# kmkolasinski/tfrecords-reader

Hardware: AMD Instinct MI355X
Metric: GiB/s + examples/s device-resident TFRecord->Feature decode, 1/2/4/8 GPU (higher is better)
Workload: dtype u8; 1 GPU; C4 directory (configs[4]) of 256 files, C1-shaped (int64 label + 12 B bytes_list id) records, 524288 +-50 % per file (default_rng(1000+f)), spec CRC-32C; this rank's LPT share (256 files) resident in HBM; records_per_gpu=134295581, framed_bytes_per_gpu=7906235019, parallelism=file-sharded x1 (LPT by bytes, no collective on the data path), batches_per_gpu=4, batch_bytes_max=1976558779, streams=2, tpl_groups_missed=0

## Files before the change

tfrecords-reader_amd/csrc/tfrg_capi.cpp:

```cpp
#include <hip/hip_runtime.h>
#include <stdlib.h>
#include <string.h>

#include <algorithm>
#include <map>
#include <numeric>
#include <string>
#include <unordered_map>
#include <vector>

#include "../../include/tfrg.h"
#include "crc32c.h"
#include "tfrg_internal.h"

namespace tfrg {
void set_error(const std::string& s);

#define HIP_TRY(expr)                                                              \
  do {                                                                             \
    hipError_t e_ = (expr);                                                        \
    if (e_ != hipSuccess) {                                                        \
      set_error(std::string(#expr) + ": " + hipGetErrorString(e_));               \
      return TFRG_E_HIP;                                                           \
    }                                                                              \
// ... 48 lines not shown
  const uint32_t* s32 = nullptr;
  const uint32_t* e32 = nullptr;
  uint32_t first = 0;
  uint32_t mode = kOffU64;
};

struct tfrg_ctx {
  int device = 0;
  hipStream_t own_stream = nullptr;
  hipStream_t last_stream = nullptr;
  uint32_t lane_max = 2048;
  uint32_t wave_stage = 0xffffffffu;
  uint64_t record_bound = 0;
  uint64_t call_bound = 0;
  int num_cus = 256;
  DBuf crc_tab, consts;
  DBuf ht, key_hash, key_off, key_blob, key_slot, slot_kind, key_w, krec;
  uint32_t n_keys = 0, n_slots = 0, ht_mask = 0;
  DBuf in_bytes, in_start, in_end;
  DBuf status, aux, verdict, order, count, loc, rs, slot_base, totals, kind_totals;
  DBuf ident;
  size_t ident_n = 0;
  DBuf i64, f32, b_off, b_len, big_list, slow_list, miss, info, tsum, crc_rec, crc_base, crc_part;
  DBuf dq, dq_cnt;
  DBuf lmask, rlist;
  DBuf bdata, boff64, blb, bbig;
  bool materialized = false;
  bool tsum_dirty = true;
  uint32_t info_slot = 0;
  bool info_clean = false;
  uint32_t n = 0;
  uint64_t cap_hint = 0;
  hipEvent_t order_ev = nullptr;
  uint64_t nbytes = 0;
  uint64_t cap_i64 = 0, cap_f32 = 0, cap_b = 0;
  bool have_result = false;
  bool rs_complete = false;
  std::unordered_map<std::string, uint32_t> key_id;
  std::vector<int32_t> key_slot_h;
  DBuf tpl;
  uint32_t n_tpl = 0;
  uint32_t tpl_w = 0;
  size_t tpl_img_off = 0;
  uint32_t tpl_img_words = 0;
  std::vector<uint32_t> tpl_h;
  bool tpl_learned = false;
  bool tpl_full = false;
  bool tpl_on = true;
  std::vector<uint8_t> slot_kind_h;
  DBuf spec;
  std::vector<uint32_t> spec_h;
  bool have_spec = false;
  bool spec_on = true;
  bool profiling = false;
  bool have_events = false;
  hipEvent_t ev[kNumStages + 1] = {};
  uint64_t hint_i64 = 0, hint_f32 = 0, hint_b = 0;
  bool hinted = false;
  bool no_hints = false;
// ... 25 lines not shown
extern "C" {

int tfrg_ctx_create(int device, tfrg_ctx** out) {
  *out = nullptr;
  int ndev = 0;
  HIP_TRY(hipGetDeviceCount(&ndev));
  if (device < 0 || device >= ndev) {
    set_error("bad device index");
    return TFRG_E_ARG;
  }
  HIP_TRY(hipSetDevice(device));
  tfrg_ctx* c = new tfrg_ctx();
  c->device = device;
  if (const char* e = getenv("TFRG_TEMPLATES")) c->tpl_on = atoi(e) != 0;
  if (const char* e = getenv("TFRG_SPEC")) c->spec_on = atoi(e) != 0;
  if (const char* e = getenv("TFRG_OPTIMISTIC")) c->optimistic_on = atoi(e) != 0;
  if (const char* e = getenv("TFRG_WALK_BESIDE")) c->walk_beside = atoi(e) != 0;
  if (const char* e = getenv("TFRG_WALK_BLOCKS")) c->walk_blocks = (uint32_t)atoi(e);
  if (const char* e = getenv("TFRG_DEBUG_POISON_LOC")) {
    char* q = const_cast<char*>(e);
    for (int i = 0; i < 4 && *q; ++i) {
      c->poison[i] = (uint32_t)strtoul(q, &q, 10);
      while (*q == ',' || *q == ' ') ++q;
    }
  }
  hipDeviceProp_t prop;
  if (hipGetDeviceProperties(&prop, device) == hipSuccess) c->num_cus = prop.multiProcessorCount;
  if (hipStreamCreateWithFlags(&c->own_stream, hipStreamNonBlocking) != hipSuccess) {
    delete c;
    set_error("hipStreamCreate failed");
    return TFRG_E_HIP;
  }
  if (hipHostMalloc(reinterpret_cast<void**>(&c->info_pin), (kInfoCount + 8) * 4) != hipSuccess) {
    (void)hipStreamDestroy(c->own_stream);
    delete c;
    set_error("hipHostMalloc failed");
    return TFRG_E_NOMEM;
  }
  std::vector<uint32_t> tab(kLeanTabOff + 32 * 256), cst(128);
  CrcTables T;
  crc_make_tables(&T);
  memcpy(tab.data(), T.t, 4096);
  uint32_t M[4][256];
  crc_make_mul_tables(gf_xpow8(1024), M);
  memcpy(tab.data() + 1024, M, 4096);
  memcpy(tab.data() + 2048, T.t, 8192);
  memcpy(tab.data() + 4096, T.t, 16384);
  for (int e = 0; e < 256; ++e)
    for (int col = 0; col < 47; ++col) tab[8192 + e * 64 + col] = T.t[(col + 1) & 15][e];
  crc_make_mul_tables(gf_xpow8(2048), M);
  memcpy(tab.data() + 24576, M, 4096);
  crc_make_mul_tables(gf_xpow8(4096), M);
  memcpy(tab.data() + 25600, M, 4096);
  for (int k = 0; k < 24; ++k) {
    crc_make_mul_tables(gf_xpow8(1024ull << k), M);
    memcpy(tab.data() + 26624 + k * 1024, M, 4096);
  }
  for (int l = 0; l < 64; ++l) cst[l] = gf_xpow8(16ull * l);
  for (int z = 0; z < 16; ++z) cst[64 + z] = gf_xpow8_inv((uint64_t)z);
  for (int k = 0; k < 32; ++k) cst[96 + k] = gf_xpow8(1024ull << k);
  for (int v = 0; v < 256; ++v) {
    uint32_t x = T.t[0][v];
    for (int d = 0; d < 32; ++d) {
      tab[kLeanTabOff + d * 256 + v] = x;
      x = (x >> 8) ^ T.t[0][x & 0xff];
    }
  }
  if (c->crc_tab.ensure(tab.size() * 4) != hipSuccess || c->consts.ensure(cst.size() * 4) != hipSuccess ||
      hipMemcpy(c->crc_tab.p, tab.data(), tab.size() * 4, hipMemcpyHostToDevice) != hipSuccess ||
      hipMemcpy(c->consts.p, cst.data(), cst.size() * 4, hipMemcpyHostToDevice) != hipSuccess) {
    set_error("constant upload failed");
    tfrg_ctx_destroy(c);
    return TFRG_E_HIP;
  }
  *out = c;
  return 0;
}

int tfrg_ctx_destroy(tfrg_ctx* c) {
  if (!c) return 0;
  (void)hipSetDevice(c->device);
  if (c->last_stream) (void)hipStreamSynchronize(c->last_stream);
// ... 164 lines not shown
  DevSchema s;
  s.n_keys = c->n_keys;
  s.n_slots = c->n_slots;
  s.ht_mask = c->ht_mask;
  s.ht = c->ht.as<uint32_t>();
  s.key_hash = c->key_hash.as<uint32_t>();
  s.key_off = c->key_off.as<uint32_t>();
  s.key_blob = c->key_blob.as<uint8_t>();
  s.key_slot = c->key_slot.as<int32_t>();
  s.slot_kind = c->slot_kind.as<uint8_t>();
  s.key_w = c->key_w.as<uint32_t>();
  s.krec = c->krec.as<uint32_t>();
  s.tpl = c->tpl.as<uint32_t>();
  s.tpl_img = s.tpl + c->tpl_img_off;
  s.tpl_img_words = c->tpl_img_words;
  s.n_tpl = c->tpl_on ? c->n_tpl : 0u;
  s.tpl_w = c->tpl_w;
  s.spec = c->spec_on && c->have_spec ? c->spec.as<uint32_t>() : nullptr;
  return s;
}

namespace {

bool tpl_hdr2(const uint8_t* p, uint32_t L, uint32_t pos, uint32_t end, uint32_t& fn, uint32_t& off, uint32_t& len) {
  if (pos >= L || (p[pos] & 0x87u) != 0x02u) return false;
  fn = (p[pos] >> 3) & 0xfu;
  uint32_t q = pos + 1, l = 0;
  for (uint32_t nb = 0;; ++nb) {
    if (nb == 3 || q >= L) return false;
    const uint32_t b = p[q++];
// ... 93 lines not shown
        mode = 1;
      }
      if (mode) {
        cw = 1u | kCountInline;
        a = c0o;
        b = c0l;
      }
    }
    t.ent.insert(t.ent.end(), {(uint32_t)slot | (mode << 24), rank, cw, a | (b << 16)});
  }
  return !t.ent.empty();
}

struct Learned {
  std::vector<uint32_t> w, spec, img;
  uint32_t W = 0;
  bool have_spec = false;
  bool full = false;
  bool ord_const = false;
  bool len_const = false;
  std::vector<uint32_t> const_len;
};
uint32_t learn_shapes(const TplSchema* c, uint32_t S, const uint8_t* h_bytes, uint64_t nbytes, const uint64_t* h_start,
                      const uint64_t* h_end, uint32_t n, uint32_t flags, Learned& out) {
  std::map<std::string, std::pair<uint32_t, Tpl>> seen;
  Tpl t;
  const uint32_t lim = n < 4096u ? n : 4096u;
  for (uint32_t j = 0; j < lim; ++j) {
    const uint32_t i = (uint32_t)((uint64_t)j * n / lim);
    uint64_t a = h_start[i], e = h_end[i];
// ... 147 lines not shown
      }
      if (k == 0) sq |= kLiQSingle;
      if ((z[2] & ~kCountInline) > 1u) sq &= ~kLiQSingle;
    }
    img[3] |= d[kLtCrcw];
    img[4] = std::min(img[4], d[kLtChain]);
    if (lut[L] == 0xffu) {
      lut[L] = (uint8_t)k;
    } else {
      uint32_t p = lut[L];
      while (img[kLiTpl + (size_t)p * tw + 2] != 0xffu) p = img[kLiTpl + (size_t)p * tw + 2];
      img[kLiTpl + (size_t)p * tw + 2] = k;
    }
  }
  memcpy(&img[kLiLut], lut.data(), lut.size());
  out.ord_const = S > 0 && S <= kLeanMaxSlots;
  for (uint32_t s2 = 0; out.ord_const && s2 < S; ++s2) {
    const uint32_t r0 = w[kLtSlot + 3 * s2] >> 16;
    out.ord_const = r0 != 0;
    for (uint32_t k = 1; out.ord_const && k < nt; ++k) out.ord_const = (w[(size_t)k * kLtWords + kLtSlot + 3 * s2] >> 16) == r0;
  }
  out.len_const = S > 0 && S <= kLeanMaxSlots;
  out.const_len.assign(S, 0u);
  for (uint32_t s2 = 0; out.len_const && s2 < S; ++s2) {
    if ((c->slot_kind[s2] & 3u) != TFRG_KIND_BYTES) continue;
    const uint32_t z0 = w[kLtSlot + 3 * s2];
    out.len_const = (z0 & 0xffu) == 3u && (z0 >> 16) != 0;
    for (uint32_t k = 1; out.len_const && k < nt; ++k) {
      const uint32_t zk = w[(size_t)k * kLtWords + kLtSlot + 3 * s2];
      out.len_const = (zk & 0xffu) == 3u && (zk >> 16) != 0 && ((zk >> 8) & 0xffu) == ((z0 >> 8) & 0xffu);
    }
    out.const_len[s2] = (z0 >> 8) & 0xffu;
  }
  out.w = std::move(w);
  out.spec = std::move(spec);
  out.img = std::move(img);
  out.W = W;
  out.have_spec = have_spec;
  return nt;
}

bool learn_single_slots(const TplSchema* c, uint32_t S, const uint8_t* h_bytes, uint64_t nbytes,
                        const uint64_t* h_start, const uint64_t* h_end, uint32_t n, uint32_t flags,
                        std::vector<uint32_t>& spec) {
  spec.assign(S ? S : 1, 0u);
  if (!S || !n) return false;
  tfrg_host_ctx* hc = nullptr;
  if (tfrg_host_ctx_create(&hc)) return false;
  std::vector<uint32_t> single(S, 0u);
  uint32_t m = 0;
  const uint32_t lim = n < 4096u ? n : 4096u;
// ... 62 lines not shown
      set_error("template allocation failed");
      return TFRG_E_NOMEM;
    }
    HIP_TRY(hipMemcpy(c->spec.p, spec.data(), (size_t)c->n_slots * 4, hipMemcpyHostToDevice));
    c->spec_h = spec;
    c->have_spec = true;
    return 0;
  }
  const uint32_t S = c->n_slots;
  const std::vector<uint32_t>& w = L.w;
  const bool have_spec = L.have_spec;
  const std::vector<uint32_t>& spec = L.spec;
  const uint32_t W = L.W;
  HIP_TRY(hipSetDevice(c->device));
  if (c->last_stream) HIP_TRY(hipStreamSynchronize(c->last_stream));
  if (c->tpl.ensure((w.size() + L.img.size()) * 4) || (have_spec && c->spec.ensure((size_t)S * 4))) {
    set_error("template allocation failed");
    return TFRG_E_NOMEM;
  }
  HIP_TRY(hipMemcpy(c->tpl.p, w.data(), w.size() * 4, hipMemcpyHostToDevice));
  HIP_TRY(hipMemcpy(c->tpl.as<uint32_t>() + w.size(), L.img.data(), L.img.size() * 4, hipMemcpyHostToDevice));
  c->tpl_img_off = w.size();
  c->tpl_img_words = (uint32_t)L.img.size();
  if (have_spec) HIP_TRY(hipMemcpy(c->spec.p, spec.data(), (size_t)S * 4, hipMemcpyHostToDevice));
  c->n_tpl = nt;
  c->tpl_w = W;
  c->tpl_h = w;
  c->spec_h = spec;
  c->have_spec = have_spec;
  c->tpl_full = L.full;
  c->ord_const = L.ord_const;
  c->len_const = L.len_const;
  c->const_len = L.const_len;
  return (int)nt;
}

extern "C" int tfrg_learn_templates_host(uint32_t n_keys, const uint8_t* key_blob, const uint64_t* key_offsets,
                                         const uint32_t* key_flags, uint32_t n_slots, const uint32_t* slot_key,
// ... 204 lines not shown
  o.info = info_cur;
  o.info_next = c->info.as<uint32_t>() + (islot ^ 1u) * kInfoCount;
  o.tsum = c->tsum.as<uint32_t>();
  o.tile_stride = tile_stride;
  o.spine_lb = reinterpret_cast<uint64_t*>(o.tsum + (size_t)S * tile_stride);
  o.n_chunks = n_chunks;
  o.irr = o.tsum + (size_t)S * tile_stride + 2ull * S * n_chunks;
  o.slow_list = c->slow_list.as<uint32_t>();
  o.crc_rec = c->crc_rec.as<uint32_t>();
  o.crc_base = c->crc_base.as<uint64_t>();
  o.crc_part = c->crc_part.as<uint64_t>();
  o.lmask = c->lmask.as<uint64_t>();
  o.rlist = c->rlist.as<uint32_t>();
  LaunchCfg cfg;
  cfg.num_cus = c->num_cus;
  cfg.lean = c->tpl_on && c->n_tpl;
  cfg.tpl_full = cfg.lean && c->tpl_full;
  cfg.spec_h = c->spec_h.empty() ? nullptr : c->spec_h.data();
  const uint64_t lane_blocks = (n + 255) / 256;
  const uint64_t lane_cap = (uint64_t)c->num_cus * 8;
  cfg.lane_grid = (int)(lane_blocks < 1 ? 1 : (lane_blocks < lane_cap ? lane_blocks : lane_cap));
  const uint64_t wave_cap = (uint64_t)c->num_cus * 4;
  const uint64_t wave_blocks = (n + 3) / 4;
  cfg.wave_grid = (int)(wave_blocks < 1 ? 1 : (wave_blocks < wave_cap ? wave_blocks : wave_cap));
  cfg.lane_max = c->lane_max;
  cfg.wave_stage = c->wave_stage;
  memcpy(cfg.poison, c->poison, sizeof(cfg.poison));
  cfg.optimistic = c->optimistic_on && !c->no_quiet && c->poison[0] == 0xffffffffu;
  cfg.walk_beside = c->walk_beside;
  cfg.walk_blocks = c->walk_blocks;
// ... 311 lines not shown
```

tfrecords-reader_amd/csrc/tfrg_internal.h:

```cpp
#pragma once
#include <stdint.h>
#include <hip/hip_runtime.h>

namespace tfrg {

struct DevSchema {
  uint32_t n_keys;
  uint32_t n_slots;
  uint32_t ht_mask;
  const uint32_t* ht;
  const uint32_t* key_hash;
  const uint32_t* key_off;
  const uint8_t* key_blob;
  const int32_t* key_slot;
  const uint8_t* slot_kind;
  const uint32_t* key_w;
  const uint32_t* krec;
  const uint32_t* tpl;
  const uint32_t* tpl_img;
  uint32_t tpl_img_words;
  uint32_t n_tpl;
  uint32_t tpl_w;
  const uint32_t* spec;
};

constexpr uint32_t kTplMaxL = 240, kTplMaxEntries = 16;
constexpr uint32_t kLtMaxW = 64;
constexpr uint32_t kLeanMaxSlots = 16;
constexpr uint32_t kLtL = 0, kLtNe = 1, kLtCrcw = 2, kLtChain = 3, kLtK = 4, kLtAbsent = 5, kLtEnt = 8,
                   kLtWin = kLtEnt + 4 * kTplMaxEntries, kLtSlot = kLtWin + 3 * kLtMaxW,
                   kLtWords = kLtSlot + 3 * kLeanMaxSlots;
constexpr uint32_t kLeanTabOff = 51200;

constexpr uint32_t kTplMaxLane = 32;
constexpr uint32_t kLiHdr = 8, kLiSlotQ = kLiHdr, kLiLut = kLiSlotQ + kLeanMaxSlots,
                   kLiLutWords = (kTplMaxL + 1 + 3) / 4, kLiTpl = (kLiLut + kLiLutWords + 3) & ~3u;
constexpr uint32_t kLiQValue = 1u << 16, kLiQSingle = 1u << 17;
__host__ __device__ constexpr uint32_t kLiTw(uint32_t W) { return 4 + 3 * W + 4 * kLeanMaxSlots; }
constexpr uint32_t kLiMaxWords = (65536u - 32768u - 512u) / 4u;

struct LeanTgt {
  uint16_t* ord;
  uint32_t* cnt;
  uint2* loc;
  uint32_t* rs;
  void* v1;
  uint32_t* v2;
  uint32_t lim;
  uint32_t kind;
  uint32_t pad[2];
};
struct LeanArgs {
  uint32_t n_tpl;
  uint32_t lane_max;
  uint32_t* tsum;
  uint32_t n_slots;
  uint32_t tile_stride;
  uint32_t img_words;
  uint32_t gpw;
  uint32_t bsplit;
  uint32_t gsplit;
  const uint8_t* finish;
  uint32_t implicit;
  LeanTgt tg[kLeanMaxSlots];
};

enum KeyRec : uint32_t { kKrHash = 0, kKrLen, kKrW0, kKrW1, kKrSlot1, kKrSlot2, kKrSlot3, kKrFlags, kKrWords };
constexpr uint32_t kLdsMaxKeys = 256;
constexpr uint32_t kLdsMaxHt = 1024;

__host__ __device__ inline uint32_t key_hash_words(uint32_t n, uint32_t w0, uint32_t w1) {
  const uint32_t a = (w0 ^ (w0 >> 11) ^ (n << 17)) & 0xffffffu;
  const uint32_t b = (w1 ^ (w1 >> 13) ^ (n << 7)) & 0xffffffu;
#if defined(__HIP_DEVICE_COMPILE__)
  uint32_t p0, p1;
  asm("v_mul_u32_u24 %0, %1, %2" : "=v"(p0) : "v"(a), "v"(0x9E3779u));
  asm("v_mul_u32_u24 %0, %1, %2" : "=v"(p1) : "v"(b), "v"(0x85EBCBu));
  uint32_t h = p0 ^ p1;
// ... 140 lines not shown
  int num_cus;
  bool lean;
  bool tpl_full;
  const uint32_t* spec_h;
  int lane_grid;
  int wave_grid;
  uint32_t lane_max;
  uint32_t wave_stage;
  bool body_count;
  uint32_t poison[4];
  bool optimistic;
  bool ran_optimistic;
  bool ord_const;
  bool len_const;
  bool ran_quiet_big;
  bool walk_beside;
  uint32_t walk_blocks;
  uint32_t implicit;
};

enum Stage : int { kStageTplLane = 0, kStageLaneCount, kStageBodyCount, kStageTailCount, kStageSpine,
                   kStageDownGather, kStageTailGather, kStageMaterialize, kNumStages };
extern const char* const kStageNames[kNumStages];

hipError_t launch_tpl_lane(const DevBatch& b, const DevOut& o, const LeanArgs& a, const uint32_t* img, uint32_t w,
                           const uint32_t* d_tab, int num_cus, hipStream_t st);
hipError_t launch_fill_placed_rows(uint32_t* rs, const uint32_t* info, uint32_t n_slots, uint32_t n, hipStream_t st);
hipError_t launch_stream_read(const void* d, uint64_t nbytes, uint32_t* sink, hipStream_t st, int variant);
hipError_t launch_decode(const DevBatch& b, const DevSchema& sc, const DevOut& o, LaunchCfg& cfg,
                         const uint32_t* d_crc_tables, const uint32_t* d_wave_consts, hipStream_t stream,
                         hipEvent_t* ev);

}
```

tfrecords-reader_amd/csrc/tfrg_kernels.hip:

```cpp
#include <hip/hip_runtime.h>
#include <algorithm>
#include <type_traits>
#include "tfrg_internal.h"
#include "crc32c.h"
#include "tfrg_walk.h"
#include "../../include/tfrg_status.h"

namespace tfrg {

#ifdef TFRG_PHASE_PROF
__device__ unsigned long long g_phase[32];
#define PHASE_MARK(t) const uint64_t t = __builtin_readcyclecounter()
#define PHASE_ADD(i, a, b) \
  do {                     \
    if (lane == 0) atomicAdd(&g_phase[i], (unsigned long long)((b) - (a))); \
  } while (0)
#else
#define PHASE_MARK(t) (void)0
#define PHASE_ADD(i, a, b) (void)0
#endif

struct Src {
  const uint8_t* buf;
  uint64_t p0;
// ... 3114 lines not shown
  const bool tail_gord = slow_tail > kLaneLdsBudget;
  const size_t tail_lds = std::max<size_t>(tail_gord ? 2048ull * 4 : slow_tail, (kTailFinishWord + 4) * 4);
  const size_t walk_lds = 256ull * kLaneSlice * 4 + S * kTailBlock * 4 + r16(S * kTailBlock * 2) + keys_lds + spec_lds;
  const bool walk_beside = quiet_big && cfg.walk_beside && walk_lds <= tail_lds;
  cfg.implicit = 0;
  DevOut ox = o;
  if (!lean) {
    ox.lmask = nullptr;
    ox.rlist = nullptr;
  }
  mark(kStageTplLane);
  if (lean) {
    LeanArgs a{};
    a.n_tpl = sc.n_tpl;
    a.img_words = sc.tpl_img_words;
    a.lane_max = cfg.lane_max;
    a.tsum = cfg.ran_optimistic ? nullptr : o.tsum;
    a.finish = cfg.ran_optimistic ? sc.slot_kind : nullptr;
    cfg.implicit = cfg.ran_optimistic ? TFRG_IMPLICIT_STATUS | (cfg.ord_const ? TFRG_IMPLICIT_ORDER : 0u) |
                                            (cfg.len_const ? TFRG_IMPLICIT_BYTES_LEN : 0u)
                                      : 0u;
    a.implicit = cfg.implicit;
    a.n_slots = (uint32_t)S;
    a.tile_stride = o.tile_stride;
    const uint64_t n = b.n;
    for (uint32_t k = 0; k < S; ++k) {
      LeanTgt& t = a.tg[k];
      t.ord = o.order + k * n;
      t.cnt = o.count + k * n;
      t.loc = o.loc + k * n;
      t.rs = o.rs + k * (n + 1);
      const uint32_t sw = scx.spec && cfg.spec_h ? cfg.spec_h[k] : 0u;
      if (sw) {
        const uint32_t kind = sw & 3u;
        const uint64_t base = n * ((sw >> 2) - 1u);
        const uint64_t cap = kind == TFRG_KIND_INT64 ? o.cap_i64 : kind == TFRG_KIND_FLOAT ? o.cap_f32 : o.cap_b;
        t.lim = cap > base ? (uint32_t)std::min<uint64_t>(cap - base, n) : 0u;
        t.kind = kind;
        if (kind == TFRG_KIND_INT64) t.v1 = o.i64 + base;
        else if (kind == TFRG_KIND_FLOAT) t.v1 = o.f32 + base;
        else t.v1 = o.b_off + base;
        t.v2 = o.b_len + base;
      }
    }
    const hipError_t e = launch_tpl_lane(b, ox, a, sc.tpl_img, sc.tpl_w, d_tab, cfg.num_cus, st);
    if (e != hipSuccess) return e;
  }
  if (cfg.ran_optimistic && !quiet_big) {
    for (int i = kStageLaneCount; i <= kStageMaterialize; ++i) mark(i);
    return hipGetLastError();
  }
  mark(kStageLaneCount);
  auto resident_grid = [&](const void* fn, size_t lds, bool cap = true) {
    int per_cu = 0;
    if (hipOccupancyMaxActiveBlocksPerMultiprocessor(&per_cu, fn, kLaneCountBlock, lds) != hipSuccess || per_cu < 1)
      per_cu = 1;
    const int g = per_cu * cfg.num_cus;
    int need = (int)(((int64_t)cfg.lane_grid * 256 + kLaneCountBlock - 1) / kLaneCountBlock);
    if (quiet) need = std::min(need, 64);
    return g < need || !cap ? g : need;
// ... 164 lines not shown
```

tfrecords-reader_amd/csrc/tfrg_tpl.hip:

```cpp
#include <hip/hip_runtime.h>
#include "tfrg_internal.h"
#include "crc32c.h"
#include "../../include/tfrg_status.h"

namespace tfrg {

namespace {

constexpr int kTplBlock = 512;
constexpr uint32_t kTplTabs = 32;
static_assert(4u * kTplTabs * 256u + 4u * kLiMaxWords + 512u <= 65536u, "lane image + CRC tables exceed LDS");
constexpr uint32_t kHitVerdict = TFRG_V_LEN_MATCH | TFRG_V_LEN_CRC | TFRG_V_DATA_CRC;

typedef __attribute__((address_space(4))) const uint32_t cu32;

__device__ __forceinline__ uint32_t rfl(uint32_t x) { return __builtin_amdgcn_readfirstlane(x); }

template <int K>
__device__ __forceinline__ uint32_t bx4(uint32_t x) {
  uint32_t r;
  const uint32_t two = 2u;
  if constexpr (K == 0)
    asm("v_lshlrev_b32_sdwa %0, %1, %2 dst_sel:DWORD dst_unused:UNUSED_PAD src0_sel:DWORD src1_sel:BYTE_0"
        : "=v"(r) : "v"(two), "v"(x));
  else if constexpr (K == 1)
    asm("v_lshlrev_b32_sdwa %0, %1, %2 dst_sel:DWORD dst_unused:UNUSED_PAD src0_sel:DWORD src1_sel:BYTE_1"
        : "=v"(r) : "v"(two), "v"(x));
  else if constexpr (K == 2)
    asm("v_lshlrev_b32_sdwa %0, %1, %2 dst_sel:DWORD dst_unused:UNUSED_PAD src0_sel:DWORD src1_sel:BYTE_2"
        : "=v"(r) : "v"(two), "v"(x));
  else
    asm("v_lshlrev_b32_sdwa %0, %1, %2 dst_sel:DWORD dst_unused:UNUSED_PAD src0_sel:DWORD src1_sel:BYTE_3"
        : "=v"(r) : "v"(two), "v"(x));
  return r;
}

__device__ __forceinline__ uint32_t xor3(uint32_t a, uint32_t b, uint32_t c) {
  return __builtin_amdgcn_bitop3_b32(a, b, c, 0x96);
}

template <int D>
__device__ __forceinline__ uint32_t tl(const uint32_t* tab, uint32_t bx) {
  return *reinterpret_cast<const uint32_t*>(reinterpret_cast<const uint8_t*>(tab) + D * 1024 + bx);
}

template <int D>
__device__ __forceinline__ uint32_t lin_word(const uint32_t* tab, uint32_t x) {
  return xor3(tl<D + 3>(tab, bx4<0>(x)), tl<D + 2>(tab, bx4<1>(x)), tl<D + 1>(tab, bx4<2>(x))) ^ tl<D>(tab, bx4<3>(x));
}

__device__ __forceinline__ uint32_t vgroups(uint32_t w, uint32_t m) {
  w &= m;
  return (w & 0x7fu) | ((w >> 1) & 0x3f80u) | ((w >> 2) & 0x1fc000u) | ((w >> 3) & 0xfe00000u);
}
__device__ __forceinline__ uint32_t bytes_mask(uint32_t nb) { return nb >= 4u ? 0xffffffffu : (1u << (nb << 3)) - 1u; }

typedef uint32_t u32x4 __attribute__((ext_vector_type(4)));

struct LaneOff {
  uint32_t s, e;
};

__device__ __forceinline__ uint32_t wave_sum(uint32_t x) {
// ... 14 lines not shown
    uint64_t acc[4] = {0, 0, 0, 0};
    for (uint32_t k = 0; k < n_slots; ++k) {
      const uint32_t kd = slot_kind[k] & 3u;
      o.slot_base[k] = acc[kd];
      acc[kd] += n;
    }
    for (int k = 0; k < 4; ++k) o.kind_totals[k] = acc[k];
    if (acc[TFRG_KIND_INT64] > o.cap_i64 || acc[TFRG_KIND_FLOAT] > o.cap_f32 || acc[TFRG_KIND_BYTES] > o.cap_b)
      o.info[kInfoOverflow] = 1u;
    const uint64_t pm = n_slots >= 64u ? ~0ull : (1ull << n_slots) - 1ull;
    o.info[kInfoPlacedLo] = (uint32_t)pm;
    o.info[kInfoPlacedHi] = (uint32_t)(pm >> 32);
  }
}

template <int W, int OM>
__global__ __launch_bounds__(kTplBlock, W == 16 ? 6 : (W == 32 ? 4 : 2)) void k_tpl_lane(
    DevBatch B, DevOut o, LeanArgs A, const uint32_t* __restrict__ img, const uint32_t* __restrict__ tabs) {
  static_assert(W == 16 || W == 32 || W == 64, "window words");
  typedef uint32_t wvec __attribute__((ext_vector_type(W)));
  __shared__ __attribute__((aligned(16))) uint32_t tab[kTplTabs * 256];
  extern __shared__ __attribute__((aligned(16))) uint32_t limg[];
  constexpr uint32_t kWaves = kTplBlock / 64;
  constexpr uint32_t kTw = kLiTw(W);
  const uint32_t lane = threadIdx.x & 63u, wib = rfl(threadIdx.x >> 6);
  cu32* gimg = (cu32*)img;
  const uint32_t crcw_u = gimg[3], chain_u = gimg[4];
  const uint8_t* lut = reinterpret_cast<const uint8_t*>(limg + kLiLut);
  const __amdgpu_buffer_rsrc_t rsrc =
      __builtin_amdgcn_make_buffer_rsrc(const_cast<uint8_t*>(B.bytes), (short)0, (int)(uint32_t)B.nbytes, 0x00020000);
  const uint32_t nb = (uint32_t)B.nbytes;
  const uint32_t ngroups = (B.n + 63u) >> 6;
  static_assert(kTileShift == 8, "4 groups of 64 records per tile");
  const bool tail = blockIdx.x >= A.bsplit;
  const uint32_t gpw = tail ? 2u : A.gpw;
  const uint32_t gbeg0 = tail ? A.gsplit + ((blockIdx.x - A.bsplit) * kWaves + wib) * 2u : (blockIdx.x * kWaves + wib) * gpw;
  const uint32_t gbeg = gbeg0 < ngroups ? gbeg0 : ngroups;
  const uint32_t gend = gbeg + gpw < ngroups ? gbeg + gpw : ngroups;
  const bool whole = (gpw & 3u) == 0u;

  auto offsets = [&](uint32_t g) -> LaneOff {
    LaneOff f{1u, 0u};
// ... 20 lines not shown
  auto in_batch = [&](uint32_t g, uint32_t s, uint32_t e) {
    return (g << 6) + lane < B.n && s <= e && e <= nb && e >= 16u;
  };
  auto window = [&](wvec& wn, const LaneOff& f) {
    const uint32_t e = f.e;
    const bool full = e >= 4u * W && e <= nb;
    const uint32_t voff = full ? e - 4u * W : 0xffffff00u;
#pragma unroll
    for (int q = 0; q < W / 4; ++q) {
      const u32x4 v = __builtin_bit_cast(u32x4, __builtin_amdgcn_raw_buffer_load_b128(rsrc, voff + 16u * q, 0, 0));
      wn[4 * q] = v.x;
      wn[4 * q + 1] = v.y;
      wn[4 * q + 2] = v.z;
      wn[4 * q + 3] = v.w;
    }
  };
  auto head_fix = [&](wvec& wn, const LaneOff& f, uint32_t g) {
    if (g != 0u) return;
    const uint32_t e = f.e;
    const bool full = e >= 4u * W && e <= nb;
    const bool head = in_batch(g, start_of(f), e) && !full;
    if (__ballot(head)) {
#pragma unroll
      for (int i = 0; i < W; ++i) {
        uint32_t x = 0;
#pragma unroll
        for (int b = 0; b < 4; ++b) {
          const int64_t p = (int64_t)e - 4 * W + 4 * i + b;
          if (head && p >= 0) x |= (uint32_t)__builtin_amdgcn_raw_buffer_load_b8(rsrc, (uint32_t)p, 0, 0) << (8 * b);
        }
// ... 28 lines not shown
      const u32x4 meta = *reinterpret_cast<const u32x4*>(tp);
      uint32_t diff = 0;
#pragma unroll
      for (int q = 0; q < W / 4; ++q) {
        const u32x4 bm = *reinterpret_cast<const u32x4*>(tp + 4 + 4 * q);
        const u32x4 mm = *reinterpret_cast<const u32x4*>(tp + 4 + W + 4 * q);
        diff |= ((w[4 * q] ^ bm.x) & mm.x) | ((w[4 * q + 1] ^ bm.y) & mm.y) | ((w[4 * q + 2] ^ bm.z) & mm.z) |
                ((w[4 * q + 3] ^ bm.w) & mm.w);
        if (q & 1) __builtin_amdgcn_sched_barrier(0);
      }
      const uint32_t* cm = tp + 4 + 2 * W;
      uint32_t c = 0;
      if (chain_u < (uint32_t)(W - 9)) {
#pragma unroll
        for (int i = 0; i < W - 9; ++i)
          if ((uint32_t)i >= chain_u) c = lin_word<0>(tab, c ^ (w[i] & cm[i]));
      }
      uint32_t lin = 0;
#define TFRG_LIN(j)                                                                                       \
  if (crcw_u & (1u << (j))) lin ^= lin_word<28 - 4 * (j)>(tab, (w[W - 9 + (j)] & cm[W - 9 + (j)]) ^ ((j) == 0 ? c : 0u));
      TFRG_LIN(0) TFRG_LIN(1) TFRG_LIN(2) TFRG_LIN(3) TFRG_LIN(4) TFRG_LIN(5) TFRG_LIN(6) TFRG_LIN(7)
#undef TFRG_LIN
      const bool ok = act && diff == 0u && crc_mask(lin ^ meta.y) == w[W - 1];
      tsel = ok ? cand : tsel;
      cand = act && !ok ? meta.z : 0xffu;
    }
    const bool hit = tsel != 0xffu;
    if (hit && !(A.implicit & TFRG_IMPLICIT_STATUS)) {
      o.status[r] = TFRG_OK;
      o.verdict[r] = (uint8_t)kHitVerdict;
    }
    if (__ballot(hit)) {
      const uint32_t* ts = limg + kLiTpl + (hit ? tsel : 0u) * kTw + 4 + 3 * W;
      for (uint32_t k = 0; k < A.n_slots; ++k) {
        const uint32_t sq = gimg[kLiSlotQ + k];
// ... 43 lines not shown
      o.lmask[g] = mm;
      if (mm) o.rlist[atomicAdd(&o.info[kInfoResid], 1u)] = g;
    }
    listed += mm ? 1u : 0u;
  };
  auto flush = [&](uint32_t g) {
    if (lane < A.n_slots && acc && A.tsum) {
      if (whole)
        A.tsum[lane * A.tile_stride + (g >> 2)] = acc;
      else
        atomicAdd(&A.tsum[lane * A.tile_stride + (g >> 2)], acc);
    }
    acc = 0;
  };
  LaneOff fa = offsets(gbeg), f0 = offsets(gbeg + 1u);
  static_assert(kTplTabs * 256u % (4u * kTplBlock) == 0u, "table copy in whole 16-byte rounds");
  constexpr uint32_t kTabRounds = kTplTabs * 256u / (4u * kTplBlock);
  u32x4 tv[kTabRounds];
#pragma unroll
  for (uint32_t j = 0; j < kTabRounds; ++j) tv[j] = reinterpret_cast<const u32x4*>(tabs)[threadIdx.x + j * kTplBlock];
  const uint32_t iw0 = threadIdx.x < A.img_words ? img[threadIdx.x] : 0u;
  wvec wa;
  window(wa, fa);
#pragma unroll
  for (uint32_t j = 0; j < kTabRounds; ++j) reinterpret_cast<u32x4*>(tab)[threadIdx.x + j * kTplBlock] = tv[j];
  if (threadIdx.x < A.img_words) limg[threadIdx.x] = iw0;
  for (uint32_t i = threadIdx.x + kTplBlock; i < A.img_words; i += kTplBlock) limg[i] = img[i];
  __syncthreads();
  for (uint32_t g = gbeg; g < gend; ++g) {
    head_fix(wa, fa, g);
    proc(wa, g, fa);
    if (((g + 1u) & 3u) == 0u || g + 1u >= gend) flush(g);
    if (g + 1u < gend) {
      window(wa, f0);
      fa = f0;
      f0 = offsets(g + 2u);
    }
  }
  if (A.finish) {
    __shared__ uint32_t s_listed[kWaves];
    __shared__ uint32_t s_last, s_total;
    if (lane == 0) s_listed[wib] = listed;
    __syncthreads();
    if (threadIdx.x == 0) {
      uint32_t mine = 0;
      for (uint32_t i = 0; i < kWaves; ++i) mine += s_listed[i];
      const uint64_t old = atomicAdd(reinterpret_cast<unsigned long long*>(o.info + kInfoTplDone),
                                     ((unsigned long long)mine << 32) | 1ull);
      s_last = (uint32_t)old == gridDim.x - 1u;
      s_total = (uint32_t)(old >> 32) + mine;
    }
    __syncthreads();
    if (s_last) tpl_quiet_finish(o, A.finish, A.n_slots, B.n, s_total);
  }
}

}

hipError_t launch_tpl_lane(const DevBatch& b, const DevOut& o, const LeanArgs& a, const uint32_t* img, uint32_t w,
                           const uint32_t* d_tab, int num_cus, hipStream_t st) {
  const uint32_t groups = (b.n + 63u) / 64u;
  const uint32_t tiles = (groups + 3u) / 4u;
  const uint32_t need = (tiles + kTplBlock / 64 - 1) / (kTplBlock / 64);
  LeanArgs a2 = a;
  a2.gpw = need < (uint32_t)num_cus / 2u ? 1u : need < (uint32_t)num_cus ? 2u : need >= 8u * (uint32_t)num_cus ? 8u : 4u;
  static const bool split_on = [] {
    const char* e = getenv("TFRG_TPL_TAIL");
    return !e || atoi(e) != 0;
  }();
  constexpr uint32_t kW = kTplBlock / 64;
  uint32_t gsplit = groups, bsplit = 0xffffffffu;
  if (split_on && a2.gpw == 8u) {
    const uint32_t small = 3u * (uint32_t)num_cus * kW * 2u;
    if (groups > 4u * small) {
      const uint32_t big_blocks = (groups - small) / (kW * a2.gpw);
      gsplit = big_blocks * kW * a2.gpw;
      bsplit = big_blocks;
    }
  }
  a2.gsplit = gsplit;
  a2.bsplit = bsplit;
  const uint32_t blocks = bsplit != 0xffffffffu
                              ? bsplit + (groups - gsplit + kW * 2u - 1u) / (kW * 2u)
                              : ((groups + a2.gpw - 1u) / a2.gpw + kW - 1u) / kW;
  const dim3 grid(blocks ? blocks : 1u);
  const uint32_t* tabs = d_tab + kLeanTabOff;
  const size_t lds = (size_t)a.img_words * 4;
#define TFRG_TPL_LAUNCH(WW, OO) hipLaunchKernelGGL((k_tpl_lane<WW, OO>), grid, dim3(kTplBlock), lds, st, b, o, a2, img, tabs)
#define TFRG_TPL_OM(WW)                                                        \
  switch (b.omode) {                                                           \
    case kOffU64: TFRG_TPL_LAUNCH(WW, kOffU64); break;                         \
    case kOffU32: TFRG_TPL_LAUNCH(WW, kOffU32); break;                         \
    default: TFRG_TPL_LAUNCH(WW, kOffEnds); break;                             \
  }
  switch (w) {
    case 16: TFRG_TPL_OM(16) break;
    case 32: TFRG_TPL_OM(32) break;
    case 64: TFRG_TPL_OM(64) break;
    default: return hipErrorInvalidValue;
  }
#undef TFRG_TPL_OM
#undef TFRG_TPL_LAUNCH
  return hipGetLastError();
}

}
```

Before: 3597 GiB/s.

## Shrink template CRC tables to used positions and stage record windows through LDS

The lane kernel previously copied 32 lean CRC tables (32 KiB) into LDS per block. Now the learner builds only the 4-table sets for CRC word positions the template actually uses, stores them after the lane image, and sizes dynamic LDS to match. For W=16 at high groups-per-wave, each wave coalesces its 64 records' byte span into a per-wave LDS staging buffer with wide buffer loads, then builds the per-lane windows by byte-aligning from LDS. This replaces scattered per-lane global loads, but adds LDS pressure and an occupancy check.

```diff
diff --git a/tfrecords-reader_amd/csrc/tfrg_capi.cpp b/tfrecords-reader_amd/csrc/tfrg_capi.cpp
--- a/tfrecords-reader_amd/csrc/tfrg_capi.cpp
+++ b/tfrecords-reader_amd/csrc/tfrg_capi.cpp
@@ -86,6 +86,8 @@
   uint64_t record_bound = 0;
   uint64_t call_bound = 0;
   int num_cus = 256;
+  uint32_t cu_lds = 65536;
+  int tpl_stage = 1;
   DBuf crc_tab, consts;
   DBuf ht, key_hash, key_off, key_blob, key_slot, slot_kind, key_w, krec;
   uint32_t n_keys = 0, n_slots = 0, ht_mask = 0;
@@ -115,6 +117,7 @@
   uint32_t tpl_w = 0;
   size_t tpl_img_off = 0;
   uint32_t tpl_img_words = 0;
+  uint32_t tpl_tab_words = 0;
   std::vector<uint32_t> tpl_h;
   bool tpl_learned = false;
   bool tpl_full = false;
@@ -170,6 +173,7 @@
   c->device = device;
   if (const char* e = getenv("TFRG_TEMPLATES")) c->tpl_on = atoi(e) != 0;
   if (const char* e = getenv("TFRG_SPEC")) c->spec_on = atoi(e) != 0;
+  if (const char* e = getenv("TFRG_TPL_STAGE")) c->tpl_stage = atoi(e);
   if (const char* e = getenv("TFRG_OPTIMISTIC")) c->optimistic_on = atoi(e) != 0;
   if (const char* e = getenv("TFRG_WALK_BESIDE")) c->walk_beside = atoi(e) != 0;
   if (const char* e = getenv("TFRG_WALK_BLOCKS")) c->walk_blocks = (uint32_t)atoi(e);
@@ -181,7 +185,10 @@
     }
   }
   hipDeviceProp_t prop;
-  if (hipGetDeviceProperties(&prop, device) == hipSuccess) c->num_cus = prop.multiProcessorCount;
+  if (hipGetDeviceProperties(&prop, device) == hipSuccess) {
+    c->num_cus = prop.multiProcessorCount;
+    if (prop.maxSharedMemoryPerMultiProcessor) c->cu_lds = (uint32_t)prop.maxSharedMemoryPerMultiProcessor;
+  }
   if (hipStreamCreateWithFlags(&c->own_stream, hipStreamNonBlocking) != hipSuccess) {
     delete c;
     set_error("hipStreamCreate failed");
@@ -193,7 +200,7 @@
     set_error("hipHostMalloc failed");
     return TFRG_E_NOMEM;
   }
-  std::vector<uint32_t> tab(kLeanTabOff + 32 * 256), cst(128);
+  std::vector<uint32_t> tab(kCrcTabWords), cst(128);
   CrcTables T;
   crc_make_tables(&T);
   memcpy(tab.data(), T.t, 4096);
@@ -215,13 +222,6 @@
   for (int l = 0; l < 64; ++l) cst[l] = gf_xpow8(16ull * l);
   for (int z = 0; z < 16; ++z) cst[64 + z] = gf_xpow8_inv((uint64_t)z);
   for (int k = 0; k < 32; ++k) cst[96 + k] = gf_xpow8(1024ull << k);
-  for (int v = 0; v < 256; ++v) {
-    uint32_t x = T.t[0][v];
-    for (int d = 0; d < 32; ++d) {
-      tab[kLeanTabOff + d * 256 + v] = x;
-      x = (x >> 8) ^ T.t[0][x & 0xff];
-    }
-  }
   if (c->crc_tab.ensure(tab.size() * 4) != hipSuccess || c->consts.ensure(cst.size() * 4) != hipSuccess ||
       hipMemcpy(c->crc_tab.p, tab.data(), tab.size() * 4, hipMemcpyHostToDevice) != hipSuccess ||
       hipMemcpy(c->consts.p, cst.data(), cst.size() * 4, hipMemcpyHostToDevice) != hipSuccess) {
@@ -416,6 +416,7 @@
   s.tpl = c->tpl.as<uint32_t>();
   s.tpl_img = s.tpl + c->tpl_img_off;
   s.tpl_img_words = c->tpl_img_words;
+  s.tpl_tab_words = c->tpl_tab_words;
   s.n_tpl = c->tpl_on ? c->n_tpl : 0u;
   s.tpl_w = c->tpl_w;
   s.spec = c->spec_on && c->have_spec ? c->spec.as<uint32_t>() : nullptr;
@@ -539,6 +540,7 @@
 
 struct Learned {
   std::vector<uint32_t> w, spec, img;
+  std::vector<uint32_t> ptab;
   uint32_t W = 0;
   bool have_spec = false;
   bool full = false;
@@ -716,6 +718,25 @@
     }
   }
   memcpy(&img[kLiLut], lut.data(), lut.size());
+  {
+    const uint32_t used = (img[3] & 0xffu) | (img[4] < W ? 0x80u : 0u);
+    uint32_t np = 0;
+    for (uint32_t j = 0; j < 8; ++j) {
+      if (!(used & (1u << j))) continue;
+      img[6 + j / 4] |= np << (8 * (j % 4));
+      out.ptab.resize((size_t)(np + 1) * kLiPtabWords);
+      uint32_t* t = &out.ptab[(size_t)np * kLiPtabWords];
+      for (uint32_t v = 0; v < 256; ++v) {
+        uint32_t x = CT.t[0][v];
+        for (uint32_t d = 0; d < 32; ++d) {
+          if (d >= 28 - 4 * j && d < 32 - 4 * j) t[(d - (28 - 4 * j)) * 256 + v] = x;
+          x = (x >> 8) ^ CT.t[0][x & 0xff];
+        }
+      }
+      ++np;
+    }
+    img[5] = np;
+  }
   out.ord_const = S > 0 && S <= kLeanMaxSlots;
   for (uint32_t s2 = 0; out.ord_const && s2 < S; ++s2) {
     const uint32_t r0 = w[kLtSlot + 3 * s2] >> 16;
@@ -737,6 +758,7 @@
   out.w = std::move(w);
   out.spec = std::move(spec);
   out.img = std::move(img);
+  out.img.resize((out.img.size() + 3) & ~(size_t)3, 0u);
   out.W = W;
   out.have_spec = have_spec;
   return nt;
@@ -829,14 +851,18 @@
   const uint32_t W = L.W;
   HIP_TRY(hipSetDevice(c->device));
   if (c->last_stream) HIP_TRY(hipStreamSynchronize(c->last_stream));
-  if (c->tpl.ensure((w.size() + L.img.size()) * 4) || (have_spec && c->spec.ensure((size_t)S * 4))) {
+  if (c->tpl.ensure((w.size() + L.img.size() + L.ptab.size()) * 4) || (have_spec && c->spec.ensure((size_t)S * 4))) {
     set_error("template allocation failed");
     return TFRG_E_NOMEM;
   }
   HIP_TRY(hipMemcpy(c->tpl.p, w.data(), w.size() * 4, hipMemcpyHostToDevice));
   HIP_TRY(hipMemcpy(c->tpl.as<uint32_t>() + w.size(), L.img.data(), L.img.size() * 4, hipMemcpyHostToDevice));
+  if (!L.ptab.empty())
+    HIP_TRY(hipMemcpy(c->tpl.as<uint32_t>() + w.size() + L.img.size(), L.ptab.data(), L.ptab.size() * 4,
+                      hipMemcpyHostToDevice));
   c->tpl_img_off = w.size();
   c->tpl_img_words = (uint32_t)L.img.size();
+  c->tpl_tab_words = (uint32_t)L.ptab.size();
   if (have_spec) HIP_TRY(hipMemcpy(c->spec.p, spec.data(), (size_t)S * 4, hipMemcpyHostToDevice));
   c->n_tpl = nt;
   c->tpl_w = W;
@@ -1071,6 +1097,8 @@
   o.rlist = c->rlist.as<uint32_t>();
   LaunchCfg cfg;
   cfg.num_cus = c->num_cus;
+  cfg.tpl_cu_lds = c->tpl_stage ? c->cu_lds : 0u;
+  cfg.tpl_stage_any = c->tpl_stage == 2;
   cfg.lean = c->tpl_on && c->n_tpl;
   cfg.tpl_full = cfg.lean && c->tpl_full;
   cfg.spec_h = c->spec_h.empty() ? nullptr : c->spec_h.data();
diff --git a/tfrecords-reader_amd/csrc/tfrg_internal.h b/tfrecords-reader_amd/csrc/tfrg_internal.h
--- a/tfrecords-reader_amd/csrc/tfrg_internal.h
+++ b/tfrecords-reader_amd/csrc/tfrg_internal.h
@@ -19,6 +19,7 @@
   const uint32_t* tpl;
   const uint32_t* tpl_img;
   uint32_t tpl_img_words;
+  uint32_t tpl_tab_words;
   uint32_t n_tpl;
   uint32_t tpl_w;
   const uint32_t* spec;
@@ -30,8 +31,9 @@
 constexpr uint32_t kLtL = 0, kLtNe = 1, kLtCrcw = 2, kLtChain = 3, kLtK = 4, kLtAbsent = 5, kLtEnt = 8,
                    kLtWin = kLtEnt + 4 * kTplMaxEntries, kLtSlot = kLtWin + 3 * kLtMaxW,
                    kLtWords = kLtSlot + 3 * kLeanMaxSlots;
-constexpr uint32_t kLeanTabOff = 51200;
-
+constexpr uint32_t kCrcTabWords = 51200;
+
+constexpr uint32_t kLiPtabWords = 4 * 256;
 constexpr uint32_t kTplMaxLane = 32;
 constexpr uint32_t kLiHdr = 8, kLiSlotQ = kLiHdr, kLiLut = kLiSlotQ + kLeanMaxSlots,
                    kLiLutWords = (kTplMaxL + 1 + 3) / 4, kLiTpl = (kLiLut + kLiLutWords + 3) & ~3u;
@@ -62,6 +64,9 @@
   uint32_t gsplit;
   const uint8_t* finish;
   uint32_t implicit;
+  uint32_t tab_words;
+  uint32_t cu_lds;
+  uint32_t stage_any;
   LeanTgt tg[kLeanMaxSlots];
 };
 
@@ -232,6 +237,8 @@
   bool ord_const;
   bool len_const;
   bool ran_quiet_big;
+  uint32_t tpl_cu_lds;
+  bool tpl_stage_any;
   bool walk_beside;
   uint32_t walk_blocks;
   uint32_t implicit;
@@ -242,7 +249,7 @@
 extern const char* const kStageNames[kNumStages];
 
 hipError_t launch_tpl_lane(const DevBatch& b, const DevOut& o, const LeanArgs& a, const uint32_t* img, uint32_t w,
-                           const uint32_t* d_tab, int num_cus, hipStream_t st);
+                           int num_cus, hipStream_t st);
 hipError_t launch_fill_placed_rows(uint32_t* rs, const uint32_t* info, uint32_t n_slots, uint32_t n, hipStream_t st);
 hipError_t launch_stream_read(const void* d, uint64_t nbytes, uint32_t* sink, hipStream_t st, int variant);
 hipError_t launch_decode(const DevBatch& b, const DevSchema& sc, const DevOut& o, LaunchCfg& cfg,
diff --git a/tfrecords-reader_amd/csrc/tfrg_kernels.hip b/tfrecords-reader_amd/csrc/tfrg_kernels.hip
--- a/tfrecords-reader_amd/csrc/tfrg_kernels.hip
+++ b/tfrecords-reader_amd/csrc/tfrg_kernels.hip
@@ -3152,6 +3152,9 @@
     LeanArgs a{};
     a.n_tpl = sc.n_tpl;
     a.img_words = sc.tpl_img_words;
+    a.tab_words = sc.tpl_tab_words;
+    a.cu_lds = cfg.tpl_cu_lds;
+    a.stage_any = cfg.tpl_stage_any ? 1u : 0u;
     a.lane_max = cfg.lane_max;
     a.tsum = cfg.ran_optimistic ? nullptr : o.tsum;
     a.finish = cfg.ran_optimistic ? sc.slot_kind : nullptr;
@@ -3181,7 +3184,7 @@
         t.v2 = o.b_len + base;
       }
     }
-    const hipError_t e = launch_tpl_lane(b, ox, a, sc.tpl_img, sc.tpl_w, d_tab, cfg.num_cus, st);
+    const hipError_t e = launch_tpl_lane(b, ox, a, sc.tpl_img, sc.tpl_w, cfg.num_cus, st);
     if (e != hipSuccess) return e;
   }
   if (cfg.ran_optimistic && !quiet_big) {
diff --git a/tfrecords-reader_amd/csrc/tfrg_tpl.hip b/tfrecords-reader_amd/csrc/tfrg_tpl.hip
--- a/tfrecords-reader_amd/csrc/tfrg_tpl.hip
+++ b/tfrecords-reader_amd/csrc/tfrg_tpl.hip
@@ -8,8 +8,9 @@
 namespace {
 
 constexpr int kTplBlock = 512;
-constexpr uint32_t kTplTabs = 32;
-static_assert(4u * kTplTabs * 256u + 4u * kLiMaxWords + 512u <= 65536u, "lane image + CRC tables exceed LDS");
+constexpr uint32_t kTplTabWords = 8;
+static_assert(4u * kTplTabWords * kLiPtabWords + 4u * kLiMaxWords + 512u <= 65536u, "lane image + CRC tables exceed LDS");
+constexpr uint32_t kStageWords = 1024 + 32, kStageRounds = (kStageWords * 4u + 1023u) / 1024u;
 constexpr uint32_t kHitVerdict = TFRG_V_LEN_MATCH | TFRG_V_LEN_CRC | TFRG_V_DATA_CRC;
 
 typedef __attribute__((address_space(4))) const uint32_t cu32;
@@ -39,14 +40,13 @@
   return __builtin_amdgcn_bitop3_b32(a, b, c, 0x96);
 }
 
-template <int D>
-__device__ __forceinline__ uint32_t tl(const uint32_t* tab, uint32_t bx) {
-  return *reinterpret_cast<const uint32_t*>(reinterpret_cast<const uint8_t*>(tab) + D * 1024 + bx);
-}
-
-template <int D>
-__device__ __forceinline__ uint32_t lin_word(const uint32_t* tab, uint32_t x) {
-  return xor3(tl<D + 3>(tab, bx4<0>(x)), tl<D + 2>(tab, bx4<1>(x)), tl<D + 1>(tab, bx4<2>(x))) ^ tl<D>(tab, bx4<3>(x));
+template <int Q>
+__device__ __forceinline__ uint32_t tl(const uint8_t* tw, uint32_t bx) {
+  return *reinterpret_cast<const uint32_t*>(tw + Q * 1024 + bx);
+}
+
+__device__ __forceinline__ uint32_t lin_word(const uint8_t* tw, uint32_t x) {
+  return xor3(tl<3>(tw, bx4<0>(x)), tl<2>(tw, bx4<1>(x)), tl<1>(tw, bx4<2>(x))) ^ tl<0>(tw, bx4<3>(x));
 }
 
 __device__ __forceinline__ uint32_t vgroups(uint32_t w, uint32_t m) {
@@ -91,18 +91,22 @@
   }
 }
 
-template <int W, int OM>
+template <int W, int OM, bool ST>
 __global__ __launch_bounds__(kTplBlock, W == 16 ? 6 : (W == 32 ? 4 : 2)) void k_tpl_lane(
     DevBatch B, DevOut o, LeanArgs A, const uint32_t* __restrict__ img, const uint32_t* __restrict__ tabs) {
   static_assert(W == 16 || W == 32 || W == 64, "window words");
+  static_assert(!ST || W == 16, "staged windows: W = 16");
   typedef uint32_t wvec __attribute__((ext_vector_type(W)));
-  __shared__ __attribute__((aligned(16))) uint32_t tab[kTplTabs * 256];
-  extern __shared__ __attribute__((aligned(16))) uint32_t limg[];
+  extern __shared__ __attribute__((aligned(16))) uint32_t tab[];
+  uint32_t* const limg = tab + A.tab_words;
   constexpr uint32_t kWaves = kTplBlock / 64;
   constexpr uint32_t kTw = kLiTw(W);
   const uint32_t lane = threadIdx.x & 63u, wib = rfl(threadIdx.x >> 6);
   cu32* gimg = (cu32*)img;
   const uint32_t crcw_u = gimg[3], chain_u = gimg[4];
+  auto tabw = [&](uint32_t j) -> const uint8_t* {
+    return reinterpret_cast<const uint8_t*>(tab) + 4u * kLiPtabWords * ((gimg[6u + (j >> 2)] >> (8u * (j & 3u))) & 0xffu);
+  };
   const uint8_t* lut = reinterpret_cast<const uint8_t*>(limg + kLiLut);
   const __amdgpu_buffer_rsrc_t rsrc =
       __builtin_amdgcn_make_buffer_rsrc(const_cast<uint8_t*>(B.bytes), (short)0, (int)(uint32_t)B.nbytes, 0x00020000);
@@ -153,6 +157,50 @@
       wn[4 * q + 2] = v.z;
       wn[4 * q + 3] = v.w;
     }
+  };
+  auto window_st = [&](wvec& wn, const LaneOff& f, uint32_t g) {
+    if constexpr (ST) {
+      uint32_t* const stg = limg + A.img_words + wib * kStageWords;
+      const uint32_t e = f.e;
+      const uint32_t g0 = g << 6;
+      const uint32_t nv = g < gend ? (B.n - g0 < 64u ? B.n - g0 : 64u) : 0u;
+      const uint32_t pe = (uint32_t)__builtin_amdgcn_update_dpp((int)e, (int)e, 0x138, 0xf, 0xf, false);
+      const bool bad = lane < nv && (e < pe || e > nb);
+      if (nv && !__ballot(bad)) {
+        const uint32_t e0 = rfl(e), hi = (uint32_t)__builtin_amdgcn_readlane((int)e, (int)(nv - 1u));
+        const uint32_t lo = (e0 >= 4u * W ? e0 - 4u * W : 0u) & ~15u;
+        const uint32_t nch = (hi - lo + 15u) >> 4;
+        if (hi > lo && nch * 16u + 4u <= kStageWords * 4u && lo + nch * 16u <= nb) {
+          u32x4 t[kStageRounds];
+#pragma unroll
+          for (uint32_t k = 0; k < kStageRounds; ++k)
+            if (lane + 64u * k < nch)
+              t[k] = __builtin_bit_cast(u32x4, __builtin_amdgcn_raw_buffer_load_b128(rsrc, lo + 16u * (lane + 64u * k), 0, 0));
+#pragma unroll
+          for (uint32_t k = 0; k < kStageRounds; ++k)
+            if (lane + 64u * k < nch) reinterpret_cast<u32x4*>(stg)[lane + 64u * k] = t[k];
+          __builtin_amdgcn_wave_barrier();
+          const bool full = e >= 4u * W && lane < nv;
+          const uint32_t b0 = full ? e - 4u * W - lo : 0u;
+          const uint32_t* const sp = stg + (b0 >> 2);
+          const uint32_t sh = b0 & 3u;
+          uint32_t prev = sp[0];
+#pragma unroll
+          for (int i = 0; i < W; ++i) {
+            const uint32_t nx = sp[i + 1];
+            wn[i] = __builtin_amdgcn_alignbyte(nx, prev, sh);
+            prev = nx;
+          }
+          __builtin_amdgcn_wave_barrier();
+          if (__ballot(!full)) {
+#pragma unroll
+            for (int i = 0; i < W; ++i) wn[i] = full ? wn[i] : 0u;
+          }
+          return;
+        }
+      }
+    }
+    window(wn, f);
   };
   auto head_fix = [&](wvec& wn, const LaneOff& f, uint32_t g) {
     if (g != 0u) return;
@@ -211,11 +259,11 @@
       if (chain_u < (uint32_t)(W - 9)) {
 #pragma unroll
         for (int i = 0; i < W - 9; ++i)
-          if ((uint32_t)i >= chain_u) c = lin_word<0>(tab, c ^ (w[i] & cm[i]));
+          if ((uint32_t)i >= chain_u) c = lin_word(tabw(7), c ^ (w[i] & cm[i]));
       }
       uint32_t lin = 0;
 #define TFRG_LIN(j)                                                                                       \
-  if (crcw_u & (1u << (j))) lin ^= lin_word<28 - 4 * (j)>(tab, (w[W - 9 + (j)] & cm[W - 9 + (j)]) ^ ((j) == 0 ? c : 0u));
+  if (crcw_u & (1u << (j))) lin ^= lin_word(tabw(j), (w[W - 9 + (j)] & cm[W - 9 + (j)]) ^ ((j) == 0 ? c : 0u));
       TFRG_LIN(0) TFRG_LIN(1) TFRG_LIN(2) TFRG_LIN(3) TFRG_LIN(4) TFRG_LIN(5) TFRG_LIN(6) TFRG_LIN(7)
 #undef TFRG_LIN
       const bool ok = act && diff == 0u && crc_mask(lin ^ meta.y) == w[W - 1];
@@ -289,16 +337,19 @@
     acc = 0;
   };
   LaneOff fa = offsets(gbeg), f0 = offsets(gbeg + 1u);
-  static_assert(kTplTabs * 256u % (4u * kTplBlock) == 0u, "table copy in whole 16-byte rounds");
-  constexpr uint32_t kTabRounds = kTplTabs * 256u / (4u * kTplBlock);
+  static_assert(kTplTabWords * kLiPtabWords % (4u * kTplBlock) == 0u, "table copy in whole 16-byte rounds");
+  constexpr uint32_t kTabRounds = kTplTabWords * kLiPtabWords / (4u * kTplBlock);
+  const uint32_t tab16 = A.tab_words >> 2;
   u32x4 tv[kTabRounds];
 #pragma unroll
-  for (uint32_t j = 0; j < kTabRounds; ++j) tv[j] = reinterpret_cast<const u32x4*>(tabs)[threadIdx.x + j * kTplBlock];
+  for (uint32_t j = 0; j < kTabRounds; ++j)
+    if (threadIdx.x + j * kTplBlock < tab16) tv[j] = reinterpret_cast<const u32x4*>(tabs)[threadIdx.x + j * kTplBlock];
   const uint32_t iw0 = threadIdx.x < A.img_words ? img[threadIdx.x] : 0u;
   wvec wa;
-  window(wa, fa);
-#pragma unroll
-  for (uint32_t j = 0; j < kTabRounds; ++j) reinterpret_cast<u32x4*>(tab)[threadIdx.x + j * kTplBlock] = tv[j];
+  window_st(wa, fa, gbeg);
+#pragma unroll
+  for (uint32_t j = 0; j < kTabRounds; ++j)
+    if (threadIdx.x + j * kTplBlock < tab16) reinterpret_cast<u32x4*>(tab)[threadIdx.x + j * kTplBlock] = tv[j];
   if (threadIdx.x < A.img_words) limg[threadIdx.x] = iw0;
   for (uint32_t i = threadIdx.x + kTplBlock; i < A.img_words; i += kTplBlock) limg[i] = img[i];
   __syncthreads();
@@ -307,7 +358,7 @@
     proc(wa, g, fa);
     if (((g + 1u) & 3u) == 0u || g + 1u >= gend) flush(g);
     if (g + 1u < gend) {
-      window(wa, f0);
+      window_st(wa, f0, g + 1u);
       fa = f0;
       f0 = offsets(g + 2u);
     }
@@ -333,7 +384,7 @@
 }
 
 hipError_t launch_tpl_lane(const DevBatch& b, const DevOut& o, const LeanArgs& a, const uint32_t* img, uint32_t w,
-                           const uint32_t* d_tab, int num_cus, hipStream_t st) {
+                           int num_cus, hipStream_t st) {
   const uint32_t groups = (b.n + 63u) / 64u;
   const uint32_t tiles = (groups + 3u) / 4u;
   const uint32_t need = (tiles + kTplBlock / 64 - 1) / (kTplBlock / 64);
@@ -359,19 +410,30 @@
                               ? bsplit + (groups - gsplit + kW * 2u - 1u) / (kW * 2u)
                               : ((groups + a2.gpw - 1u) / a2.gpw + kW - 1u) / kW;
   const dim3 grid(blocks ? blocks : 1u);
-  const uint32_t* tabs = d_tab + kLeanTabOff;
-  const size_t lds = (size_t)a.img_words * 4;
-#define TFRG_TPL_LAUNCH(WW, OO) hipLaunchKernelGGL((k_tpl_lane<WW, OO>), grid, dim3(kTplBlock), lds, st, b, o, a2, img, tabs)
-#define TFRG_TPL_OM(WW)                                                        \
+  const uint32_t* tabs = img + a.img_words;
+  size_t lds = ((size_t)a.tab_words + a.img_words) * 4;
+  const size_t lds_st = lds + (size_t)kW * kStageWords * 4;
+  const bool staged = w == 16 && (a2.gpw >= 8u || a.stage_any) && lds_st + 64u <= 65536u &&
+                      3u * ((lds_st + 64u + 2047u) & ~(size_t)2047u) <= a.cu_lds;
+  if (staged) lds = lds_st;
+#define TFRG_TPL_LAUNCH(WW, OO, SS) \
+  hipLaunchKernelGGL((k_tpl_lane<WW, OO, SS>), grid, dim3(kTplBlock), lds, st, b, o, a2, img, tabs)
+#define TFRG_TPL_OM(WW, SS)                                                    \
   switch (b.omode) {                                                           \
-    case kOffU64: TFRG_TPL_LAUNCH(WW, kOffU64); break;                         \
-    case kOffU32: TFRG_TPL_LAUNCH(WW, kOffU32); break;                         \
-    default: TFRG_TPL_LAUNCH(WW, kOffEnds); break;                             \
+    case kOffU64: TFRG_TPL_LAUNCH(WW, kOffU64, SS); break;                     \
+    case kOffU32: TFRG_TPL_LAUNCH(WW, kOffU32, SS); break;                     \
+    default: TFRG_TPL_LAUNCH(WW, kOffEnds, SS); break;                         \
   }
   switch (w) {
-    case 16: TFRG_TPL_OM(16) break;
-    case 32: TFRG_TPL_OM(32) break;
-    case 64: TFRG_TPL_OM(64) break;
+    case 16:
+      if (staged) {
+        TFRG_TPL_OM(16, true)
+      } else {
+        TFRG_TPL_OM(16, false)
+      }
+      break;
+    case 32: TFRG_TPL_OM(32, false) break;
+    case 64: TFRG_TPL_OM(64, false) break;
     default: return hipErrorInvalidValue;
   }
 #undef TFRG_TPL_OM
```

Result: faster. 4115 GiB/s (median of 6 runs) (+14.4%).
